# MiRaCLeXeoN/sduss

Measured on AMD Instinct MI355X. Metric: images/sec (node), SDXL 1024^2 50-step, fixed prompt, CFG, higher is better.
Workload: dtype bf16; 1 GPU; SDXL-base-1.0 UNet 1024x1024 50-step Euler, CFG 5.0, 4 requests/step (denoiser batch 8) per GPU, is_sliced=False, random-init weights of the real architecture (2.57 B params), one data-parallel replica per GPU, no collective; resolution=1024, steps_per_image=50

## Files before the change

include/mxdenoise.h:

```cpp
#ifndef MXDENOISE_H
#define MXDENOISE_H

#include <stddef.h>
#include <stdint.h>

#ifdef __cplusplus
extern "C" {
#endif

enum { MX_F32 = 0, MX_F16 = 1, MX_BF16 = 2 };

const char* mx_last_error(void);
int mx_version(void);
#define MX_PROF_KINDS 12
int mx_profile_enable(int on);
int mx_profile_collect(double* out);
int mx_profile_records(double* out, int max_records);

size_t mx_groupnorm_halo_workspace_bytes(int N, int C, int cpg);
int mx_groupnorm_halo(void* stream, const void* x, const void* gamma, const void* beta, void* y,
                      int N, int C, int H, int W, int cpg, double eps, int padding,
                      const int32_t* latent_offset, int n_latents, const int32_t* patch_map,
                      const int32_t* padding_idx, int dtype, void* workspace);
int mx_halo_only(void* stream, const void* x, void* y, int N, int C, int H, int W,
// ... 65 lines not shown
  float ln_eps;
  float* stats_out;
  const mx_gemm_seg* segs;
  int n_segs;
  int splitk;
  const float* ln_final;
  float* ln_final_out;
  unsigned* ln_final_cnt;
  float* gn_part_out;
  int cin_valid;
} mx_gemm_desc;

int mx_gemm(void* stream, const mx_gemm_desc* d);
int mx_gemm_launches(const mx_gemm_desc* d);
int mx_gemm_stats_slabs(const mx_gemm_desc* d);
int mx_gemm_ln_prefers_pass(const mx_gemm_desc* d);
int mx_gemm_ln_final_supported(const mx_gemm_desc* d);
int mx_gemm_gn_partials_supported(const mx_gemm_desc* d, int conv);
enum { MX_LN_ROUTES_PATCH_PARALLEL = 1, MX_LN_ROUTES_PATCH_CACHE = 2, MX_LN_ROUTES_TICKETS = 4 };
int mx_unet_ln_routes(int M, int C, int layers, int n_groups, int flags, int routes[4]);
enum { MX_FORM_TILE_GENERIC = 0, MX_FORM_TILE_256 = 1, MX_FORM_TILE_128 = 2, MX_FORM_PERSISTENT_256 = 3, MX_FORM_SMALL_M = 4, MX_FORM_CONV_SMALL_N = 5, MX_FORM_CONV_SMALL_CIN = 6 };
int mx_gemm_form(const mx_gemm_desc* d, int conv);
int mx_gemm_kernel_name(const mx_gemm_desc* d, int conv, int launch, char* buf, int cap);
int mx_gemm_kernel_names(char* buf, int cap);
int mx_attention_kernel_name(int B, int H, int Lq, int Lk, int ldo, int prescaled, int causal, int bias, int key_chunk, int force_cross, char* buf, int cap);
int mx_attention_kernel_names(char* buf, int cap);
#define MX_STATS_PITCH(slabs) (((slabs) + 3) & ~3)
int mx_row_stats(void* stream, const void* x, int ldx, float* stats, int M, int C);
int mx_conv3x3(void* stream, const mx_gemm_desc* d);
int mx_conv3x3_halo_serves(const mx_gemm_desc* d);
int mx_conv3x3_halo(void* stream, const mx_gemm_desc* d);
int mx_conv3x3_halfrow_serves(const mx_gemm_desc* d);
int mx_conv3x3_halfrow(void* stream, const mx_gemm_desc* d);
int mx_gemm_splitk(const mx_gemm_desc* d, int conv);
void mx_gemm_release_scratch(void* stream, int all);

#define MX_VT_POS(key) (((key) & ~12) | (((key) & 4) << 1) | (((key) & 8) >> 1))
#define MX_VT_LD(Lk) (((Lk) + 15) / 16 * 16)

int mx_attention(void* stream, const void* q, int ldq, const void* k, int ldk, const void* vt, int ldvt,
                 int64_t vt_batch_stride, void* o, int ldo, int B, int H, int Lq, int Lk, float scale);
#define MX_ATTN_QSCALE(scale) ((scale) * 1.4426950408889634f)
int mx_attention_prescaled(void* stream, const void* q, int ldq, const void* k, int ldk, const void* vt, int ldvt,
                           int64_t vt_batch_stride, void* o, int ldo, int B, int H, int Lq, int Lk);
int mx_attention_cross_prescaled(void* stream, const void* q, int ldq, const void* k, int ldk, const void* vt, int ldvt,
                                 int64_t vt_batch_stride, void* o, int ldo, int B, int H, int Lq, int Lk);
typedef struct mx_attn_problem {
  const void* q; const void* k; const void* vt; void* o;
  int64_t vt_batch_stride;
  int B, Lq, Lk, ldvt;
} mx_attn_problem;
int mx_attention_prescaled_grouped(void* stream, const mx_attn_problem* probs, int n, int ldq, int ldk, int ldo, int H);
int mx_attention_prescaled_bias(void* stream, const void* q, int ldq, const void* k, int ldk, const void* vt, int ldvt,
                                int64_t vt_batch_stride, void* o, int ldo, int B, int H, int Lq, int Lk, const float* bias, int ldb);
int mx_attention_prescaled_causal(void* stream, const void* q, int ldq, const void* k, int ldk, const void* vt, int ldvt,
                                  int64_t vt_batch_stride, void* o, int ldo, int B, int H, int L);

int mx_layernorm(void* stream, const void* x, void* y, const float* gamma, const float* beta,
                 int M, int C, float eps);

int mx_rmsnorm(void* stream, const void* x, void* y, const float* w, int M, int C, float eps);

int mx_layernorm_mod(void* stream, const void* x, void* y, void* y2, const float* scale, const float* shift,
                     const float* scale2, const float* shift2, int ldmod, int M, int C, int rows_per_batch, float eps);
int mx_layernorm_mod_grouped(void* stream, const void* x, void* y, void* y2, const float* scale, const float* shift, const float* scale2,
                             const float* shift2, int ldmod, int C, float eps, const int* batches, const int* rows_per_batch, int n);
// ... 378 lines not shown
```

sduss_amd/csrc/gemm_args.h:

```cpp
#pragma once
#include "common.h"
#include "../../include/mxdenoise.h"

namespace mx {

constexpr int kMaxSegs = MX_MAX_SEGS;
struct GemmSeg {
  const bf16_t* a; const bf16_t* a2; void* c; const bf16_t* residual; bf16_t* vt; const float* rowbias; const float* gate;
  const float* ln_stats; float* stats_out;
  int M, tile0, rows_per_batch, ldvt;
  int B, Hin, Win, Hout, Wout;
  int a_batch_rows, a_row_off, c_batch_rows, c_row_off;
};

struct GemmArgs {
  const bf16_t* a;
  const bf16_t* w;
  void* c;
  const float* bias;
  const float* rowbias;
  const bf16_t* residual;
  bf16_t* vt;
  int M, N, K;
  int lda, ldc, ldr, ldrb;
// ... 401 lines not shown
  const int band = local / band_tiles;
  const int r = local - band * band_tiles;
  const int rows = (mloc - band * MB) < MB ? (mloc - band * MB) : MB;
  tn = r / rows;
  tm = ((band * MB + (r - tn * rows)) << 3) + xcd;
}

__device__ __forceinline__ void lane_exchange_pair(float (&a)[4], float (&b)[4]) {
#pragma unroll
  for (int d = 0; d < 4; ++d) {
    unsigned x = __float_as_uint(a[d]), y = __float_as_uint(b[d]);
    auto r = __builtin_amdgcn_permlane32_swap(x, y, false, false);
    auto t = __builtin_amdgcn_permlane16_swap(r[0], r[1], false, false);
    a[d] = __uint_as_float(t[0]);
    b[d] = __uint_as_float(t[1]);
  }
}

__device__ __forceinline__ u32x4 lane_xor1(const u32x4 x) {
  u32x4 r;
#pragma unroll
  for (int d = 0; d < 4; ++d) r[d] = (unsigned)__builtin_amdgcn_update_dpp(0, (int)x[d], 0xB1, 0xF, 0xF, true);
  return r;
}

constexpr int EPI_F_QKV = 1;
constexpr int EPI_F_ACT = 2;
constexpr int EPI_F_ALL = 3;
constexpr int EPI_F_TANH = 4;
__host__ __device__ inline int gemm_epi_features(int flags) {
  const int acts = flags & (MX_EPI_SILU | MX_EPI_GELU | MX_EPI_GELU_TANH | MX_EPI_QUICK_GELU | MX_EPI_GEGLU_TANH);
  return ((flags & MX_EPI_QKV) ? EPI_F_QKV : 0) | (acts == 0 ? 0 : acts == MX_EPI_GELU_TANH ? EPI_F_TANH : EPI_F_ACT);
}
template <int NI, int MI, bool GEGLU, bool VEC = true, bool VPF = true, bool STATS = true, int FEAT = EPI_F_ALL, bool EMIT = STATS, bool RSTD_LOAD = false>
__device__ __forceinline__ void gemm_epilogue_regs(const GemmArgs& p, f32x4 (&acc)[NI][MI], const int m_wave0, const int wave_n0,
                                                   const int fr, const int fq, const float (&ln_rstd_a)[MI]) {
#pragma clang fp contract(off)
  constexpr int NIO = GEGLU ? NI / 2 : NI;
  constexpr int NP = NIO / 2;
  constexpr bool ODD = (NIO & 1) != 0;
  constexpr int DEPTH = MI <= 4 ? MI : 2;
  static_assert(!GEGLU || NI % 4 == 0, "GEGLU: hidden and gate halves must be whole pairs");
  const int flags = p.flags;
  constexpr bool ACT = (FEAT & EPI_F_ACT) != 0;
  constexpr bool TANH = (FEAT & (EPI_F_ACT | EPI_F_TANH)) != 0;
  const bool qkv = (FEAT & EPI_F_QKV) != 0 && (flags & MX_EPI_QKV) != 0;
  int seg_idx = 0, seg_grp = 0, seg_pos = 0;
  bool to_vt = false;
  if (qkv) {
    seg_idx = wave_n0 / p.seg;
    seg_grp = seg_idx / p.period;
    seg_pos = seg_idx - seg_grp * p.period;
    to_vt = seg_pos == p.period - 1;
  }
  const bool rms = qkv && (flags & MX_EPI_RMSNORM) && !to_vt;
  const float w_scale = (!rms && p.out_scale != 0.f && (!qkv || seg_pos == 0)) ? p.out_scale : 1.0f;
  const int col0 = GEGLU ? wave_n0 / 2 : qkv ? seg_grp * (p.period - 1) * p.seg + seg_pos * p.seg + (wave_n0 - seg_idx * p.seg) : wave_n0;
  const bool has_res = !GEGLU && p.residual != nullptr;
  const bool has_rb = VEC && !GEGLU && p.rowbias != nullptr, has_gate = VEC && !GEGLU && p.gate != nullptr;

  f32x4 bias_r[NI];
#pragma unroll
  for (int i = 0; i < NI; ++i) {
    bias_r[i] = f32x4{0.f, 0.f, 0.f, 0.f};
    if (p.bias && (GEGLU || i < NIO)) bias_r[i] = *reinterpret_cast<const f32x4*>(p.bias + wave_n0 + i * 16 + fq * 4);
  }
  f32x4 rmsw_r[NI];
  if (rms) {
    const float* w = seg_pos == 0 ? p.rms_wq : p.rms_wk;
// ... 27 lines not shown
#pragma unroll
          for (int i = 0; i < NIO; ++i) {
            const f32x4 t = STATS ? fma4(acc[i][j], rs, bias_r[i]) : acc[i][j] + bias_r[i];
#pragma unroll
            for (int q = 0; q < 4; ++q) dst[(long)(i * 16 + q) * p.ldvt] = f32_to_bf16(t[q]);
          }
        }
        rv += 16;
        if (rv >= rpb_v) { rv -= rpb_v; ++bv; }
      }
      return;
    }
  }
  const bool odd_lane = (fr & 1) != 0;
  const int rpb = p.rows_per_batch > 0 ? p.rows_per_batch : 0x7fffffff;
  const int cbr = p.c_batch_rows > 0 ? p.c_batch_rows : (p.rows_per_batch > 0 ? p.rows_per_batch : 0);
  const int cro = p.c_batch_rows > 0 ? p.c_row_off : 0;
  const int b_last = p.rows_per_batch > 0 ? (p.M - 1) / p.rows_per_batch : 0;
  const int r_last = p.M - 1 - b_last * (p.rows_per_batch > 0 ? p.rows_per_batch : 0);
  const int row_last = b_last * cbr + cro + r_last;
  const int mA0 = (m_wave0 + fr) & ~1;
  int row_a[MI], row_b[MI];
  int bo_walk = 0, ro_walk = 0;
  {
    int bA = p.rows_per_batch > 0 ? mA0 / p.rows_per_batch : 0;
    int rA = mA0 - bA * (p.rows_per_batch > 0 ? p.rows_per_batch : 0);
#pragma unroll
    for (int j = 0; j < MI; ++j) {
      int bB = bA, rB = rA + 1;
      if (rB >= rpb) { rB = 0; ++bB; }
      const int mA = mA0 + 16 * j;
      row_a[j] = mA < p.M ? bA * cbr + cro + rA : row_last;
      row_b[j] = mA + 1 < p.M ? bB * cbr + cro + rB : row_last;
      if constexpr (VEC) { if (j == 0) { bo_walk = odd_lane ? bB : bA; ro_walk = odd_lane ? rB : rA; } }
      rA += 16;
      if (rA >= rpb) { rA -= rpb; ++bA; }
    }
  }
  auto token = [&](int j) __attribute__((always_inline)) { return m_wave0 + j * 16 + fr; };
  auto row_own = [&](int j) __attribute__((always_inline)) { return odd_lane ? row_b[j] : row_a[j]; };
  const char* const res_base = reinterpret_cast<const char*>(p.residual);
  char* const c_base = reinterpret_cast<char*>(p.c);
  const unsigned ldr_b = (unsigned)p.ldr * 2u, ldc_b = (unsigned)p.ldc * 2u;
  auto res_at = [&](int row, int col) __attribute__((always_inline)) { return res_base + (unsigned long long)(unsigned)row * ldr_b + (unsigned)(col * 2); };
  auto c_at = [&](int row, int col) __attribute__((always_inline)) { return c_base + (unsigned long long)(unsigned)row * ldc_b + (unsigned)(col * 2); };
  auto store_c16 = [&](int row, int col, const u32x4 v) __attribute__((always_inline)) { *reinterpret_cast<u32x4*>(c_at(row, col)) = v; };
  auto store_c8 = [&](int row, int col, const u32x2 v) __attribute__((always_inline)) { *reinterpret_cast<u32x2*>(c_at(row, col)) = v; };

  auto load_res = [&](int j, int pr) __attribute__((always_inline)) -> u32x4 {
    if (!has_res) return u32x4{0u, 0u, 0u, 0u};
    return *reinterpret_cast<const u32x4*>(res_at(row_own(j), col0 + pr * 32 + fq * 8));
  };
  auto load_res_odd = [&](int j) __attribute__((always_inline)) -> u32x2 {
    if (!has_res) return u32x2{0u, 0u};
    return *reinterpret_cast<const u32x2*>(res_at(row_own(j), col0 + NP * 32 + fq * 4));
  };
  f32x4 rb_r[VEC ? NIO : 1], gate_r[VEC ? NIO : 1];
  auto load_batch_vectors = [&](int j) __attribute__((always_inline)) {
    if constexpr (VEC) {
      (void)j;
      const int bidx = bo_walk < b_last ? bo_walk : b_last;
      ro_walk += 16;
      if (ro_walk >= rpb) { ro_walk -= rpb; ++bo_walk; }
#pragma unroll
      for (int i = 0; i < NIO; ++i) {
        const int n = wave_n0 + i * 16 + fq * 4;
// ... 187 lines not shown
```

sduss_amd/csrc/gemm_dispatch.cpp:

```cpp
#include <algorithm>
#include <cstdlib>

#include <mutex>
#include <unordered_map>

#include "common.h"
#include "../../include/mxdenoise.h"
#include "gemm_args.h"
#include "gemm_forms.h"

namespace mx {

int launch_generic(hipStream_t s, const GemmArgs& a, int form);
int launch_v2(hipStream_t s, const GemmArgs& a, int form);
int launch_v5(hipStream_t s, const GemmArgs& a, int form);
int launch_v4(hipStream_t s, const GemmArgs& a, int form);
int launch_small_m(hipStream_t s, const GemmArgs& a, int form);
int launch_conv_small_n(hipStream_t s, const GemmArgs& a, int form);
int launch_conv_small_cin(hipStream_t s, const GemmArgs& a, int form);
bool small_m_serves(const mx_gemm_desc* d, bool conv);
int small_m_form(long N, long K, int flags);
bool conv_small_n_serves(const mx_gemm_desc* d);
bool conv_small_cin_serves(const mx_gemm_desc* d);

// ... 497 lines not shown
  for (const auto& s : kNotFaster) if (d->Win == s[0] && d->Cin == s[1] && d->N == s[2]) return 0;
  return conv_halo_lds_bytes(d->Win, false);
}

static int conv_halfrow_serves(const mx_gemm_desc* d) {
  if (!conv_staged_common(d) || d->Win != 128 || d->Hin % 4 != 0) return 0;
  return conv_halo_lds_bytes(d->Win, true);
}

static int run_conv_halo(void* stream, const mx_gemm_desc* d, bool half_rows) {
  MX_CHECK(d != nullptr, "conv3x3_halo: null descriptor");
  if (half_rows) MX_CHECK(conv_halfrow_serves(d) > 0, "conv3x3_halfrow: the descriptor is not served (mx_conv3x3_halfrow_serves); run mx_conv3x3");
  else MX_CHECK(conv_halo_serves(d) > 0, "conv3x3_halo: the descriptor is not served (mx_conv3x3_halo_serves); run mx_conv3x3");
  if (int rc = validate(d, true)) return rc;
  MX_CHECK(!d->stats_out && !d->ln_final_out, "conv3x3_halo: no row statistics");
  if (d->gn_part_out)
    MX_CHECK(!d->residual && (!d->rowbias || d->rows_per_batch % 64 == 0) && ((uintptr_t)d->gn_part_out & 15) == 0,
             "conv3x3_halo: gn_part_out needs an epilogue of bias (+ row bias) only and 16-byte alignment");
  GemmRoute r;
  r.bn = 160; r.rows = 256;
  GemmArgs a;
  fill_args(d, true, r, a);
  hipStream_t s = (hipStream_t)stream;
  if (prof_enabled()) {
    const double kk = 9.0 * d->Cin, Mt = (double)d->M;
    prof_begin(s, PROF_CONV_V2_160, 2.0 * Mt * (double)d->N * kk, 2.0 * (Mt * d->Cin + (double)d->N * d->K + Mt * d->N), d->M, d->N, (int)kk);
  }
  MX_CHECK(launch_conv_halo(s, a, d->rowbias != nullptr, half_rows) == 0, "conv3x3_halo: no instantiation for this image width");
  prof_end(s);
  MX_LAUNCH_CHECK();
  return 0;
}

}

extern "C" int mx_conv3x3_halo_serves(const mx_gemm_desc* d) { return mx::conv_halo_serves(d); }
extern "C" int mx_conv3x3_halo(void* stream, const mx_gemm_desc* d) { return mx::run_conv_halo(stream, d, false); }
extern "C" int mx_conv3x3_halfrow_serves(const mx_gemm_desc* d) { return mx::conv_halfrow_serves(d); }
extern "C" int mx_conv3x3_halfrow(void* stream, const mx_gemm_desc* d) { return mx::run_conv_halo(stream, d, true); }
extern "C" int mx_gemm(void* stream, const mx_gemm_desc* d) { return mx::run(stream, d, false); }
extern "C" int mx_conv3x3(void* stream, const mx_gemm_desc* d) { return mx::run(stream, d, true); }
extern "C" void mx_gemm_release_scratch(void* stream, int all) { mx::splitk_release((hipStream_t)stream, all != 0); }

extern "C" int mx_gemm_launches(const mx_gemm_desc* d) { mx::GemmPlan p; return mx::plan_of(d, false, p) ? p.n : 1; }
extern "C" int mx_gemm_form(const mx_gemm_desc* d, int conv) { mx::GemmPlan p; return mx::plan_of(d, conv != 0, p) ? (int)p.r[0].family : MX_FORM_TILE_GENERIC; }
extern "C" int mx_gemm_splitk(const mx_gemm_desc* d, int conv) { mx::GemmPlan p; return mx::plan_of(d, conv != 0, p) ? p.r[0].splitk : 0; }
extern "C" int mx_gemm_gn_partials_supported(const mx_gemm_desc* d, int conv) { mx::GemmPlan p; return mx::plan_of(d, conv != 0, p) && p.r[0].gn_part; }
extern "C" int mx_gemm_stats_slabs(const mx_gemm_desc* d) { mx::GemmPlan p; return mx::plan_of_variant(d, true, p) ? p.r[0].stats_slabs : 0; }
extern "C" int mx_gemm_ln_final_supported(const mx_gemm_desc* d) { mx::GemmPlan p; return mx::plan_of_variant(d, true, p) && p.r[0].ln_final_out; }
extern "C" int mx_gemm_ln_prefers_pass(const mx_gemm_desc* d) { mx::GemmPlan p; return mx::plan_of_variant(d, false, p) && p.r[0].bn == 256; }
extern "C" int mx_gemm_kernel_name(const mx_gemm_desc* d, int conv, int launch, char* buf, int cap) {
  mx::GemmPlan p;
  if (launch < 0 || !mx::plan_of(d, conv != 0, p)) return -1;
  if (launch >= p.n) return 0;
  if (p.r[launch].form < 0) return -1;
  return mx::copy_name(mx::kGemmKernelNames[p.r[launch].form], buf, cap);
}
extern "C" int mx_gemm_kernel_names(char* buf, int cap) { return mx::join_names(mx::kGemmKernelNames, mx::GK_COUNT, buf, cap); }
```

sduss_amd/csrc/unet_sdxl.cpp:

```cpp
#include <hip/hip_runtime.h>

#include <algorithm>
#include <cstring>
#include <functional>
#include <map>
#include <string>
#include <vector>

#include "../../include/mxdenoise.h"
#include "common.h"
#include "graph_cache.h"
#include "ln_route.h"
#include "patch_cache.h"
#include "plan_base.h"

namespace mx {
int launch_prep_latent(hipStream_t s, const void* in, int dtype, void* out, int B, int Cin, int HW, int CP);
int launch_nhwc_to_nchw(hipStream_t s, const void* in, void* out, int dtype, int B, int C, int HW, int ld);
int launch_time_embed(hipStream_t s, const float* timesteps, const void* text_embeds, const float* time_ids,
                      void* tsin, void* addin, int B, int d0, int text_dim, int da);
int launch_concat(hipStream_t s, const void* a, const void* b, void* out, long M, int C1, int C2);
size_t gn_workspace_exact(int B, int H, int W, int C, int patch);
int launch_sq_diff_partial(hipStream_t s, const void* a, const void* b, long elems_per_sample, int B, double* partial, const int* slot = nullptr);
int launch_gn_pp_partial(hipStream_t s, const void* x, int C1, const void* x2, int B, int H, int W, int C, int groups, void* workspace, double* sums);
// ... 2 lines not shown
                        const double* fresh_own = nullptr, int own_rank = 0);
}
extern "C" int mx_attention_prescaled_chunked(void* stream, const void* q, int ldq, const void* k, int ldk, const void* vt, int ldvt,
                                              int64_t vt_batch_stride, void* o, int ldo, int B, int H, int Lq, int Lk, int key_chunk,
                                              int64_t k_batch_stride, int64_t k_chunk_stride, int64_t vt_chunk_stride);

using mx::bf16_t;
using mx::LnVia;

struct mx_unet {
  mx_unet_config cfg;
  mx::WeightTable weights;
  mx::GraphCache graphs;
  mx::PinnedBuf skip_pin;
  std::map<std::vector<long>, std::vector<size_t>> pp_sizes;
  struct CtxEntry {
    uint64_t key = 0; int B = 0, ctx_len = 0; bool valid = false; uint64_t stamp = 0;
    std::vector<bf16_t*> k, vt; std::vector<size_t> k_bytes, vt_bytes;
    hipEvent_t ev = nullptr; hipStream_t last = nullptr; bool recorded = false;
  };
  uint64_t ctx_key = 0;
  std::vector<CtxEntry> ctx_store;
  uint64_t ctx_clock = 0;
  long ctx_hits = 0, ctx_misses = 0;
  void ctx_clear() {
    for (auto& e : ctx_store) {
      if (e.last) (void)hipStreamSynchronize(e.last);
      for (auto* q : e.k) if (q) (void)hipFree(q);
      for (auto* q : e.vt) if (q) (void)hipFree(q);
      if (e.ev) (void)hipEventDestroy(e.ev);
    }
    ctx_store.clear();
  }
  ~mx_unet() { ctx_clear(); }
};

namespace {

constexpr int kConvInPad = 64;

static std::vector<std::pair<int, int>> kv_widths(const mx_unet_config& c) {
  const int nlev = c.n_levels;
  std::vector<std::pair<int, int>> widths;
  auto add = [&](int dim, int n) { for (auto& wv : widths) if (wv.first == dim) { wv.second += n; return; } widths.push_back({dim, n}); };
  for (int i = 0; i < nlev; ++i) if (c.down_has_attn[i]) add(c.block_out_channels[i], c.layers_per_block * c.transformer_layers[i]);
  add(c.block_out_channels[nlev - 1], c.transformer_layers[nlev - 1]);
  for (int i = 0; i < nlev; ++i) { const int lv = nlev - 1 - i; if (c.down_has_attn[lv]) add(c.block_out_channels[lv], (c.layers_per_block + 1) * c.transformer_layers[lv]); }
  return widths;
}

struct RowStats { float* buf = nullptr; int slabs = 0; float* fin = nullptr; unsigned* cnt = nullptr; };
struct Linear {
  const bf16_t* a; int lda; std::string stem; void* c; int ldc; int M, N, K;
  const void* residual = nullptr; int ldr = 0; int flags = 0; float out_scale = 0.f;
  const bf16_t* a2 = nullptr; int lda2 = 0;
  const RowStats* ln = nullptr; LnVia ln_via = LnVia::Pass;
  RowStats* stats_out = nullptr; LnVia stats_via = LnVia::Pass;
  Linear& plus(const void* r, int ld) { residual = r; ldr = ld; return *this; }
  Linear& epilogue(int f) { flags = f; return *this; }
  Linear& scaled(float s) { out_scale = s; return *this; }
  Linear& concat(const bf16_t* x2, int ld2) { a2 = x2; lda2 = ld2; return *this; }
  Linear& folded_ln(const RowStats& st, LnVia via) { ln = &st; ln_via = via; return *this; }
  Linear& leaves_stats(RowStats& st, LnVia via) { stats_out = &st; stats_via = via; return *this; }
};
struct ConvIn { bf16_t* t = nullptr; bf16_t* padded = nullptr; };
struct Conv {
  ConvIn in; int Hin, Win, Cin; std::string prefix; bf16_t* out; int Cout;
  int stride = 1, up = 0, corner_patch = 0;
// ... 251 lines not shown
    d.corner_patch = c.corner_patch;
    d.M = gB[0] * d.Hout * d.Wout; d.N = Cout; d.K = 9 * Cin;
    d.rowbias = c.rowbias; d.ldrb = c.ldrb; d.rows_per_batch = d.Hout * d.Wout;
    d.residual = c.residual; d.ldr = Cout;
    mx_gemm_seg sg[MX_MAX_SEGS];
    if (ng > 1) {
      std::memset(sg, 0, sizeof(sg));
      long in0 = 0, out0 = 0;
      for (int g = 0; g < ng; ++g) {
        mx_gemm_seg& q = sg[g];
        q.B = gB[g]; q.Hin = ch[g]; q.Win = cw[g];
        q.Hout = ((ch[g] << up) + stride - 1) / stride; q.Wout = ((cw[g] << up) + stride - 1) / stride;
        q.M = gB[g] * q.Hout * q.Wout; q.rows_per_batch = q.Hout * q.Wout;
        q.a = x + in0 * Cin; q.c = c.out + out0 * Cout;
        q.residual = c.residual ? (const bf16_t*)c.residual + out0 * Cout : nullptr;
        q.rowbias = c.rowbias ? c.rowbias + (long)gb0[g] * c.ldrb : nullptr;
        in0 += (long)gB[g] * ch[g] * cw[g]; out0 += q.M;
      }
      d.segs = sg; d.n_segs = ng;
    }
    if (c.gn_part && c.gn_done && ng == 1 && mx_gemm_gn_partials_supported(&d, 1)) { d.gn_part_out = c.gn_part; *c.gn_done = true; }
    d.cin_valid = conv_cin_valid;
    if (mx_conv3x3_halo_serves(&d) && mx_gemm_form(&d, 1) == MX_FORM_TILE_256) {
      if (!ok()) return false;
      if (quiet()) return true;
      if (mx_conv3x3_halo(stream, &d)) return fail(std::string("conv3x3_halo: ") + mx_last_error());
      return true;
    }
    if (mx_conv3x3_halfrow_serves(&d) && mx_gemm_form(&d, 1) == MX_FORM_TILE_256) {
      if (!ok()) return false;
      if (quiet()) return true;
      if (mx_conv3x3_halfrow(stream, &d)) return fail(std::string("conv3x3_halfrow: ") + mx_last_error());
      return true;
    }
    return gemm(d, true);
  }
  bool groupnorm(const bf16_t* x, bf16_t* y, const std::string& prefix, int h, int wd, int C, float eps, bool silu, int patch,
                 const bf16_t* x2 = nullptr, int C1 = 0) {
    if (!ok()) return false;
    const size_t m = ar.mark();
    mx_gn_problem pr[MX_MAX_SEGS];
    long r0 = 0;
    for (int k = 0; k < ng; ++k) {
      pr[k].x = x + r0 * (x2 ? C1 : C); pr[k].x2 = x2 ? x2 + r0 * (C - C1) : nullptr; pr[k].y = y + r0 * C;
      pr[k].B = gB[k]; pr[k].H = ch[k]; pr[k].W = cw[k];
      r0 += (long)gB[k] * ch[k] * cw[k];
    }
    const size_t need = ng > 1 ? mx_groupnorm_nhwc_grouped_workspace_bytes(pr, ng, C) : mx::gn_workspace_exact(gB[0], h, wd, C, patch);
    void* ws = ar.alloc(need);
    if (!ws) return fail("workspace too small");
    const float* g = wf(prefix + ".weight", C); const float* b = wf(prefix + ".bias", C);
    if (ok() && !quiet()) {
      if (mx_groupnorm_nhwc_grouped(stream, pr, ng, x2 ? C1 : C, g, b, C, u->cfg.norm_num_groups, eps, silu ? 1 : 0, patch, ws))
        fail(std::string("groupnorm: ") + mx_last_error());
    }
    ar.release(m);
    return ok();
  }
  bool groupnorm_from_partials(const bf16_t* x, bf16_t* y, const std::string& prefix, int h, int wd, int C, float eps, bool silu, const float* part,
                               const float* add_bias, const float* add_rowbias, int ldrb) {
    if (!ok()) return false;
    const size_t m = ar.mark();
    void* ws = ar.alloc(mx::gn_workspace_exact(gB[0], h, wd, C, 0));
    if (!ws) return fail("workspace too small");
    const float* g = wf(prefix + ".weight", C); const float* b = wf(prefix + ".bias", C);
    if (ok() && !quiet()) {
// ... 729 lines not shown
extern "C" mx_unet* mx_unet_create(const mx_unet_config* cfg) {
  if (check_cfg(cfg)) return nullptr;
  mx_unet* u = new mx_unet();
  u->cfg = *cfg;
  return u;
}

extern "C" void mx_unet_destroy(mx_unet* u) { delete u; }

extern "C" int mx_unet_ln_routes(int M, int C, int layers, int n_groups, int flags, int routes[4]) {
  MX_CHECK(routes != nullptr && C > 0 && C % 64 == 0 && layers > 0 && n_groups >= 1 && n_groups <= MX_MAX_SEGS && M >= n_groups, "unet_ln_routes: bad arguments");
  const mx::LnRoutes r = mx::ln_routes(mx::LnRows::even(M, n_groups), C, layers, (flags & MX_LN_ROUTES_PATCH_PARALLEL) != 0, (flags & MX_LN_ROUTES_PATCH_CACHE) != 0,
                                       (flags & MX_LN_ROUTES_TICKETS) != 0);
  routes[0] = (int)r.norm1; routes[1] = (int)r.norm2; routes[2] = (int)r.norm3; routes[3] = r.norm3_from_merge ? 1 : 0;
  return 0;
}

extern "C" int mx_unet_set_context_key(mx_unet* u, uint64_t key) {
  MX_CHECK(u != nullptr, "unet_set_context_key: null handle");
  u->ctx_key = key;
  return 0;
}
extern "C" int mx_unet_context_stats(const mx_unet* u, long* hits, long* misses) {
  MX_CHECK(u != nullptr, "unet_context_stats: null handle");
  if (hits) *hits = u->ctx_hits;
  if (misses) *misses = u->ctx_misses;
  return 0;
}

extern "C" int mx_unet_set_weights(mx_unet* u, const void* blob, uint64_t blob_bytes, const mx_weight_entry* table, int n) {
  MX_CHECK(u != nullptr, "unet_set_weights: null handle");
  u->graphs.clear();
  u->ctx_clear();
  return u->weights.set("unet_set_weights", blob, blob_bytes, table, n);
}

extern "C" size_t mx_unet_workspace_bytes(const mx_unet* u, int batch, int H, int W, int ctx_len) {
  if (!u) return 0;
  size_t best = 0;
  const int div = 1 << (u->cfg.n_levels - 1);
  for (int gp : {0, 2 * div}) {
    if (gp > 0 && (H % gp != 0 || W % gp != 0 || gp >= H)) continue;
    size_t peak = 0;
    mx::ForwardCall c = dry_call(batch, H, W, ctx_len);
    c.gn_patch = gp; c.peak = &peak;
    if (forward_impl(u, c)) return 0;
    best = std::max(best, peak);
  }
  return best + 4096;
}

extern "C" int mx_unet_validate(const mx_unet* u, int batch, int H, int W, int ctx_len) {
  MX_CHECK(u && u->weights.blob, "unet_validate: weights not set");
  mx::ForwardCall c = dry_call(batch, H, W, ctx_len);
  c.lookup = true;
  return forward_impl(u, c);
}

extern "C" int mx_unet_forward(mx_unet* u, void* stream, const void* latents, int io_dtype, const float* timesteps,
                               const void* ehs, const void* text_embeds, const float* time_ids, void* out, int batch, int H,
                               int W, int ctx_len, int gn_patch, void* workspace, size_t workspace_bytes) {
  mx::ForwardCall c = forward_call(stream, io_dtype, timesteps, ehs, text_embeds, time_ids, ctx_len, workspace, workspace_bytes);
  c.latents = latents; c.out = out; c.batch = batch; c.H = H; c.W = W; c.gn_patch = gn_patch;
  return forward_impl(u, c);
}

extern "C" size_t mx_unet_workspace_bytes_mixed(const mx_unet* u, const mx_unet_group* groups, int n_groups, int ctx_len) {
// ... 233 lines not shown
```

sduss_amd/lib.py:

```python
from __future__ import annotations

import ctypes as C
import os
from typing import Optional

_HERE = os.path.dirname(os.path.abspath(__file__))
LIB_PATH = os.path.join(_HERE, "libmxdenoise.so")

MX_F32, MX_F16, MX_BF16 = 0, 1, 2
EPI_SILU, EPI_GEGLU, EPI_OUT_F32, EPI_QKV, EPI_GELU_TANH, EPI_RES_BCAST, EPI_RMSNORM, EPI_GELU, EPI_QUICK_GELU, EPI_GEGLU_TANH = 1, 2, 4, 8, 16, 32, 64, 128, 256, 512


class MxError(RuntimeError):
    """Raised for every non-zero status of the C ABI (the reference's launcher only printed
    cudaGetLastError and went on -- norm_silu_concat.cu:434-437; SURVEY.md section 8b asks to raise)."""


MAX_SEGS = 4


class GemmSeg(C.Structure):
    _fields_ = [
        ("a", C.c_void_p), ("a2", C.c_void_p), ("c", C.c_void_p), ("residual", C.c_void_p), ("vt", C.c_void_p), ("rowbias", C.c_void_p),
        ("gate", C.c_void_p), ("ln_stats", C.c_void_p), ("stats_out", C.c_void_p),
# ... 164 lines not shown
    _fields_ = [("kind", C.c_void_p), ("coef", C.c_void_p), ("hist", C.c_void_p)]


LORA_NO_VECTOR = (1 << 64) - 1
LORA_MAX_RANK = 512


class LoraTerm(C.Structure):
    _fields_ = [("w_off", C.c_uint64), ("N", C.c_int), ("K", C.c_int), ("row0", C.c_int), ("rows", C.c_int), ("up", C.c_void_p),
                ("down_t", C.c_void_p), ("R", C.c_int), ("scale", C.c_float), ("colsum_off", C.c_uint64), ("bias_off", C.c_uint64),
                ("dbias", C.c_void_p)]


class WeightEntry(C.Structure):
    _fields_ = [("name", C.c_char_p), ("offset", C.c_uint64), ("bytes", C.c_uint64)]


_vp, _i, _f, _d, _i64, _sz = C.c_void_p, C.c_int, C.c_float, C.c_double, C.c_int64, C.c_size_t
SYMBOLS = {
    "mx_last_error": (C.c_char_p, []),
    "mx_version": (_i, []),
    "mx_profile_enable": (_i, [_i]),
    "mx_profile_collect": (_i, [C.POINTER(C.c_double)]),
    "mx_profile_records": (_i, [C.POINTER(C.c_double), _i]),
    "mx_groupnorm_halo_workspace_bytes": (_sz, [_i, _i, _i]),
    "mx_groupnorm_halo": (_i, [_vp, _vp, _vp, _vp, _vp, _i, _i, _i, _i, _i, _d, _i, _vp, _i, _vp, _vp, _i, _vp]),
    "mx_halo_only": (_i, [_vp, _vp, _vp, _i, _i, _i, _i, _vp, _i]),
    "mx_gemm": (_i, [_vp, C.POINTER(GemmDesc)]),
    "mx_conv3x3": (_i, [_vp, C.POINTER(GemmDesc)]),
    "mx_conv3x3_halo": (_i, [_vp, C.POINTER(GemmDesc)]),
    "mx_conv3x3_halo_serves": (_i, [C.POINTER(GemmDesc)]),
    "mx_conv3x3_halfrow": (_i, [_vp, C.POINTER(GemmDesc)]),
    "mx_conv3x3_halfrow_serves": (_i, [C.POINTER(GemmDesc)]),
    "mx_gemm_stats_slabs": (_i, [C.POINTER(GemmDesc)]),
    "mx_gemm_ln_prefers_pass": (_i, [C.POINTER(GemmDesc)]),
    "mx_row_stats": (_i, [_vp, _vp, _i, _vp, _i, _i]),
    "mx_attention": (_i, [_vp, _vp, _i, _vp, _i, _vp, _i, _i64, _vp, _i, _i, _i, _i, _i, _f]),
    "mx_attention_prescaled": (_i, [_vp, _vp, _i, _vp, _i, _vp, _i, _i64, _vp, _i, _i, _i, _i, _i]),
    "mx_attention_cross_prescaled": (_i, [_vp, _vp, _i, _vp, _i, _vp, _i, _i64, _vp, _i, _i, _i, _i, _i]),
    "mx_layernorm": (_i, [_vp, _vp, _vp, _vp, _vp, _i, _i, _f]),
    "mx_groupnorm_nhwc_workspace_bytes": (_sz, [_i, _i, _i, _i]),
    "mx_groupnorm_nhwc": (_i, [_vp, _vp, _vp, _vp, _vp, _i, _i, _i, _i, _i, _f, _i, _i, _vp]),
    "mx_groupnorm_nhwc_cat": (_i, [_vp, _vp, _i, _vp, _vp, _vp, _vp, _i, _i, _i, _i, _i, _f, _i, _i, _vp]),
    "mx_attention_prescaled_grouped": (_i, [_vp, C.POINTER(AttnProblem), _i, _i, _i, _i, _i]),
    "mx_groupnorm_nhwc_grouped_workspace_bytes": (_sz, [C.POINTER(GnProblem), _i, _i]),
    "mx_groupnorm_nhwc_grouped": (_i, [_vp, C.POINTER(GnProblem), _i, _i, _vp, _vp, _i, _i, _f, _i, _i, _vp]),
    "mx_unet_workspace_bytes_mixed": (_sz, [_vp, C.POINTER(UNetGroup), _i, _i]),
    "mx_unet_forward_mixed": (_i, [_vp, _vp, C.POINTER(UNetGroup), _i, _i, _vp, _vp, _vp, _vp, _i, _i, _vp, _sz]),
    "mx_unet_forward_mixed_trace": (_i, [_vp, _vp, C.POINTER(UNetGroup), _i, _i, _vp, _vp, _vp, _vp, _i, _i, _vp, _sz, C.c_char_p, _vp, _sz]),
    "mx_mmdit_workspace_bytes_mixed": (_sz, [_vp, C.POINTER(UNetGroup), _i, _i]),
    "mx_mmdit_forward_mixed": (_i, [_vp, _vp, C.POINTER(UNetGroup), _i, _i, _vp, _vp, _vp, _i, _vp, _sz]),
    "mx_unet_create": (_vp, [C.POINTER(UNetConfigC)]),
    "mx_unet_destroy": (None, [_vp]),
    "mx_unet_set_context_key": (_i, [_vp, C.c_uint64]),
    "mx_unet_context_stats": (_i, [_vp, C.POINTER(C.c_long), C.POINTER(C.c_long)]),
    "mx_unet_set_weights": (_i, [_vp, _vp, C.c_uint64, C.POINTER(WeightEntry), _i]),
    "mx_unet_workspace_bytes": (_sz, [_vp, _i, _i, _i, _i]),
    "mx_unet_validate": (_i, [_vp, _i, _i, _i, _i]),
    "mx_unet_forward": (_i, [_vp, _vp, _vp, _i, _vp, _vp, _vp, _vp, _vp, _i, _i, _i, _i, _i, _vp, _sz]),
    "mx_forest_predict": (_i, [_vp, _vp, _vp, _vp, _vp, _vp, _i, _vp, _i, _i, _vp]),
    "mx_skip_counters_bytes": (_sz, [_i, _i, _i]),
    "mx_skip_decide_host": (_i, [C.POINTER(DeviceForestC), _i, _i, _i, _i, _vp, _vp, _vp, _vp, _vp, _vp, _vp, _vp, _vp]),
    "mx_skip_decide_device": (_i, [_vp, C.POINTER(SkipDecideArgs)]),
    "mx_pc_image_copy": (_i, [_vp, _vp, _vp, _vp, _i, _i, _i, _i64, _i, _vp, _i, _vp, _i64, _i]),
    "mx_pc_rows_load_stats": (_i, [_vp, _vp, _vp, _vp, _i, _i, _i, _i64, _vp, _vp, _vp, _f, _i64]),
    "mx_pc_gather": (_i, [_vp, _vp, _i, _i, _vp, _vp, _i, _vp, _i, _i, _i, _i, _i]),
# ... 184 lines not shown
```

Before: 1.493 images/s.

## Fuse nearest-2x upsample into 3x3 conv via per-phase folded weights

Adds a conv kernel for the upsampler convolutions that works on the low-resolution input. Nearest 2x upsampling followed by a 3x3 conv is rewritten as four output phases, each with pre-summed weights. The summed weights are packed once at weight load with bf16 hi/lo splits to keep precision, giving 7 slices instead of 9 and avoiding the upsampled intermediate. The new path costs extra device memory for packed weights, a special epilogue row mapping that scatters to interleaved output rows, and a separate kernel with its own pipelining.

```diff
diff --git a/include/mxdenoise.h b/include/mxdenoise.h
--- a/include/mxdenoise.h
+++ b/include/mxdenoise.h
@@ -121,6 +121,10 @@
 int mx_conv3x3_halo(void* stream, const mx_gemm_desc* d);
 int mx_conv3x3_halfrow_serves(const mx_gemm_desc* d);
 int mx_conv3x3_halfrow(void* stream, const mx_gemm_desc* d);
+size_t mx_conv3x3_up2_pack_bytes(int N, int Cin);
+int mx_conv3x3_up2_pack(void* stream, const void* w, int N, int Cin, void* wp);
+int mx_conv3x3_up2_serves(const mx_gemm_desc* d);
+int mx_conv3x3_up2(void* stream, const mx_gemm_desc* d, const void* wp);
 int mx_gemm_splitk(const mx_gemm_desc* d, int conv);
 void mx_gemm_release_scratch(void* stream, int all);
 
diff --git a/sduss_amd/csrc/conv_up2.hip b/sduss_amd/csrc/conv_up2.hip
--- /dev/null
+++ b/sduss_amd/csrc/conv_up2.hip
@@ -0,0 +1,258 @@
+#include "common.h"
+#include "../../include/mxdenoise.h"
+#include "gemm_args.h"
+#include "gemm_dma_loader.h"
+
+#include <type_traits>
+
+#ifndef MX_UP2_PHASE_SLOWEST
+#define MX_UP2_PHASE_SLOWEST 0
+#endif
+
+namespace mx {
+
+constexpr int UP2_BN = 160;
+constexpr int UP2_SLICES = 7;
+constexpr int UP2_WSTAGE_BYTES = UP2_BN * DMA_BK * 2;
+constexpr int UP2_ZERO_BYTES = 256;
+__host__ __device__ constexpr int up2_lines(int W) { return (256 / W + 2) * W; }
+__host__ __device__ constexpr int up2_xbuf_bytes(int W) { return up2_lines(W) * DMA_BK * 2; }
+__host__ __device__ constexpr int up2_lds_bytes(int W) { return 2 * up2_xbuf_bytes(W) + 3 * UP2_WSTAGE_BYTES + UP2_ZERO_BYTES; }
+__host__ __device__ constexpr int up2_slice_of_piece(int XN, int i) { return (i * 5) / (XN - 1); }
+__host__ __device__ constexpr int up2_pieces_in_slice(int XN, int T) {
+  int n = 0;
+  for (int i = 0; i < XN; ++i) n += up2_slice_of_piece(XN, i) == T ? 1 : 0;
+  return n;
+}
+
+__global__ __launch_bounds__(256) void up2_pack_kernel(const bf16_t* __restrict__ w, bf16_t* __restrict__ wp, const int N, const int Cin) {
+  const long idx = (long)blockIdx.x * 256 + threadIdx.x;
+  if (idx >= (long)N * Cin) return;
+  const int n = (int)(idx / Cin), c = (int)(idx - (long)n * Cin);
+  float t[3][3];
+#pragma unroll
+  for (int kh = 0; kh < 3; ++kh)
+#pragma unroll
+    for (int kw = 0; kw < 3; ++kw) t[kh][kw] = bf16_to_f32(w[(long)n * 9 * Cin + (long)(kh * 3 + kw) * Cin + c]);
+#pragma unroll
+  for (int ph = 0; ph < 4; ++ph) {
+    const int a = ph >> 1, b = ph & 1;
+    const int kho = a ? 2 : 0, kh0 = a ? 0 : 1, kh1 = kh0 + 1;
+    const int kwo = b ? 2 : 0, kw0 = b ? 0 : 1, kw1 = kw0 + 1;
+    const float sv = t[kho][kw0] + t[kho][kw1];
+    const float sh = t[kh0][kwo] + t[kh1][kwo];
+    const float sc = ((t[kh0][kw0] + t[kh0][kw1]) + t[kh1][kw0]) + t[kh1][kw1];
+    bf16_t* dst = wp + ((long)ph * N + n) * (UP2_SLICES * (long)Cin) + c;
+    const bf16_t vh = f32_to_bf16(sv), hh = f32_to_bf16(sh), ch = f32_to_bf16(sc);
+    dst[0] = f32_to_bf16(t[kho][kwo]);
+    dst[1 * (long)Cin] = vh; dst[2 * (long)Cin] = f32_to_bf16(sv - bf16_to_f32(vh));
+    dst[3 * (long)Cin] = hh; dst[4 * (long)Cin] = f32_to_bf16(sh - bf16_to_f32(hh));
+    dst[5 * (long)Cin] = ch; dst[6 * (long)Cin] = f32_to_bf16(sc - bf16_to_f32(ch));
+  }
+}
+
+int launch_up2_pack(hipStream_t s, const void* w, int N, int Cin, void* wp) {
+  const long n = (long)N * Cin;
+  hipLaunchKernelGGL(up2_pack_kernel, dim3((unsigned)((n + 255) / 256)), dim3(256), 0, s, (const bf16_t*)w, (bf16_t*)wp, N, Cin);
+  return 0;
+}
+
+template <int W>
+__global__ __launch_bounds__(512, 2) void conv_up2_kernel(const GemmArgs pk) {
+  constexpr int BN = UP2_BN, MI = 4, NI = BN / 32;
+  constexpr int LINES = up2_lines(W);
+  constexpr int XBUF = up2_xbuf_bytes(W);
+  constexpr int XN = LINES * 8 / 512;
+  constexpr int WCH = BN * 8, WI = 3;
+  constexpr int WRING = 2 * XBUF, ZERO = WRING + 3 * UP2_WSTAGE_BYTES;
+  static_assert(W == 32 || W == 64, "a tile is whole low-resolution rows of 32 or 64 pixels");
+  static_assert(up2_lds_bytes(W) <= 160 * 1024, "LDS of one workgroup");
+  static_assert(LINES * 8 % 512 == 0 && XBUF % 256 == 0, "whole DMA instructions; buffers keep the bank half of a line");
+  static_assert(up2_slice_of_piece(XN, XN - 1) == 5, "the last piece is issued one load phase before the chunk's last");
+  __shared__ __attribute__((aligned(256))) char smem[up2_lds_bytes(W)];
+
+  const GemmArgs& p = pk;
+  const int mt = p.M / 256, nt = p.N / BN;
+  int ph, bt;
+  {
+    const int b = blockIdx.x;
+    if (MX_UP2_PHASE_SLOWEST) { ph = b / (mt * nt); bt = b - ph * (mt * nt); }
+    else if ((mt & 7) != 0) { ph = b & 3; bt = b >> 2; }
+    else { const int local = b >> 3; ph = local & 3; bt = ((local >> 2) << 3) | (b & 7); }
+  }
+  int tm, tn;
+  gemm_tile_of_block(bt, mt, nt, p.xcd_map, tm, tn);
+  const int pa = ph >> 1, pb = ph & 1;
+  const int tid = threadIdx.x;
+  const int lane = tid & 63;
+  const int wave = __builtin_amdgcn_readfirstlane(tid >> 6);
+  const int wm = wave >> 1;
+  const int wn = wave & 1;
+  const bool group_b = wave >= 4;
+  const int cs = tid & 7;
+  const int nchunks = p.Cin / DMA_BK;
+  const char* zero = reinterpret_cast<const char*>(g_zero_page);
+
+  const int m0 = tm * 256, n0 = tn * BN;
+  const int hw = p.Hin * p.Win;
+  const int img = m0 / hw;
+  const int y0 = (m0 - img * hw) / W;
+  const char* xsrc[XN];
+#pragma unroll
+  for (int i = 0; i < XN; ++i) {
+    const int P = (i * 512 + tid) >> 3;
+    const int sr = P / W, x = P - sr * W;
+    const int iy = y0 - 1 + sr;
+    const bool ok = iy >= 0 && iy < p.Hin;
+    const long off = (((long)img * p.Hin + iy) * W + x) * (long)p.Cin * 2;
+    xsrc[i] = (ok ? reinterpret_cast<const char*>(p.a) + off : zero) + swz(P, cs) * 16;
+  }
+  const long w_row = UP2_SLICES * (long)p.Cin;
+  const char* wsrc[WI];
+#pragma unroll
+  for (int i = 0; i < WI; ++i) {
+    int q = i * 512 + tid;
+    if (q >= WCH) q -= WCH;
+    const int row = q >> 3;
+    wsrc[i] = reinterpret_cast<const char*>(p.w) + (((long)ph * p.N + n0 + row) * w_row + swz(row, cs) * 8) * 2;
+  }
+  const long w_slice_step = (long)p.Cin * 2, w_chunk_step = DMA_BK * 2 - (UP2_SLICES - 1) * (long)p.Cin * 2;
+
+  auto issue_x = [&](int buf, int i) __attribute__((always_inline)) {
+    glds16(xsrc[i], smem + buf * XBUF + (i * 512 + wave * 64) * 16);
+  };
+  auto advance_x = [&](int next_chunk) __attribute__((always_inline)) {
+#pragma unroll
+    for (int i = 0; i < XN; ++i) xsrc[i] = next_chunk < nchunks ? xsrc[i] + DMA_BK * 2 : zero + lane * 16;
+  };
+  auto issue_w = [&](int stage) __attribute__((always_inline)) {
+#pragma unroll
+    for (int i = 0; i < WI; ++i) {
+      const int qb = (i * 512 + wave * 64 >= WCH) ? i * 512 + wave * 64 - WCH : i * 512 + wave * 64;
+      glds16(wsrc[i], smem + WRING + stage * UP2_WSTAGE_BYTES + qb * 16);
+    }
+  };
+  auto step_w = [&](long step) __attribute__((always_inline)) {
+#pragma unroll
+    for (int i = 0; i < WI; ++i) wsrc[i] += step;
+  };
+  auto to_next_chunk_w = [&](bool last) __attribute__((always_inline)) {
+#pragma unroll
+    for (int i = 0; i < WI; ++i) wsrc[i] = last ? zero + lane * 16 : wsrc[i] + w_chunk_step;
+  };
+
+  const int fr = lane & 15;
+  const int fq = lane >> 4;
+  unsigned wrd[2];
+  unsigned xrd[3][2];
+  unsigned zrd[3][2];
+#pragma unroll
+  for (int ks = 0; ks < 2; ++ks) {
+    const int wrow = wn * (BN / 2) + fr;
+    wrd[ks] = (unsigned)(WRING + wrow * 128 + swz(wrow, ks * 4 + fq) * 16);
+#pragma unroll
+    for (int d = 0; d < 3; ++d) {
+      const int line = wm * 64 + fr + d - 1;
+      const int key = ((fr + d - 1) >> 1) & 7;
+      const int rel = line * 128 + ((ks * 4 + fq) ^ key) * 16;
+      xrd[d][ks] = (unsigned)rel;
+      zrd[d][ks] = (unsigned)(ZERO + (rel & 255));
+    }
+  }
+  const bool lane_left = fr == 0, lane_right = fr == 15;
+
+  if (tid < UP2_ZERO_BYTES / 16) *reinterpret_cast<u32x4*>(smem + ZERO + tid * 16) = u32x4{0u, 0u, 0u, 0u};
+
+#pragma unroll
+  for (int i = 0; i < XN; ++i) issue_x(0, i);
+  advance_x(1);
+  issue_w(0); step_w(w_slice_step);
+  issue_w(1); step_w(w_slice_step);
+  wait_vmcnt<WI>();
+
+  f32x4 acc[NI][MI];
+#pragma unroll
+  for (int i = 0; i < NI; ++i)
+#pragma unroll
+    for (int j = 0; j < MI; ++j) acc[i][j] = f32x4{0.f, 0.f, 0.f, 0.f};
+  float ln_rstd[MI];
+#pragma unroll
+  for (int j = 0; j < MI; ++j) ln_rstd[j] = 1.0f;
+  asm volatile("s_waitcnt lgkmcnt(0)" ::: "memory");
+  MX_BAR();
+  if (group_b) MX_BAR();
+
+  const unsigned yoff_o = (unsigned)((pa ? 2 : 0) * W * 128), yoff_s = (unsigned)(W * 128);
+  int stage = 0;
+
+  auto run = [&](auto pbc) __attribute__((always_inline)) {
+    constexpr bool PB = decltype(pbc)::value;
+    for (int cc = 0; cc < nchunks; ++cc) {
+      const int cur = cc & 1, nxt = cur ^ 1;
+      const unsigned xb = (unsigned)(cur * XBUF);
+      const bool last = cc + 1 == nchunks;
+      auto phase = [&](auto tc) __attribute__((always_inline)) {
+        constexpr int T = decltype(tc)::value;
+        constexpr int dx = (T == 0 || T == 3 || T == 4) ? (PB ? 1 : -1) : 0, d = dx + 1;
+        constexpr int NX = up2_pieces_in_slice(XN, T);
+        const unsigned xrow = xb + (T < 3 ? yoff_o : yoff_s);
+        const unsigned wst = (unsigned)(stage * UP2_WSTAGE_BYTES);
+        bf16x8 wf[2][NI], xf[2][MI];
+#pragma unroll
+        for (int ks = 0; ks < 2; ++ks) {
+#pragma unroll
+          for (int i = 0; i < NI; ++i) wf[ks][i] = *reinterpret_cast<const bf16x8*>(smem + wrd[ks] + wst + i * (16 * 128));
+#pragma unroll
+          for (int j = 0; j < MI; ++j) {
+            unsigned a = xrow + xrd[d][ks] + (unsigned)(j * (16 * 128));
+            if (dx == -1 && (j * 16) % W == 0) a = lane_left ? zrd[d][ks] : a;
+            if (dx == 1 && (j * 16 + 16) % W == 0) a = lane_right ? zrd[d][ks] : a;
+            xf[ks][j] = *reinterpret_cast<const bf16x8*>(smem + a);
+          }
+        }
+#pragma unroll
+        for (int i = 0; i < XN; ++i)
+          if (up2_slice_of_piece(XN, i) == T) issue_x(nxt, i);
+        const int st2 = stage == 0 ? 2 : stage - 1;
+        issue_w(st2);
+        stage = stage == 2 ? 0 : stage + 1;
+        if (T == 4) to_next_chunk_w(last);
+        else step_w(T > 4 && last ? 0 : w_slice_step);
+        if (T == UP2_SLICES - 1) advance_x(cc + 2);
+        wait_vmcnt<WI + NX>();
+        asm volatile("s_waitcnt lgkmcnt(0)" ::: "memory");
+        __builtin_amdgcn_sched_barrier(0);
+        MX_BAR();
+        __builtin_amdgcn_s_setprio(1);
+#pragma unroll
+        for (int ks = 0; ks < 2; ++ks)
+#pragma unroll
+          for (int i = 0; i < NI; ++i)
+#pragma unroll
+            for (int j = 0; j < MI; ++j) acc[i][j] = __builtin_amdgcn_mfma_f32_16x16x32_bf16(wf[ks][i], xf[ks][j], acc[i][j], 0, 0, 0);
+        __builtin_amdgcn_s_setprio(0);
+        MX_BAR();
+      };
+      phase(std::integral_constant<int, 0>{}); phase(std::integral_constant<int, 1>{}); phase(std::integral_constant<int, 2>{});
+      phase(std::integral_constant<int, 3>{}); phase(std::integral_constant<int, 4>{}); phase(std::integral_constant<int, 5>{});
+      phase(std::integral_constant<int, 6>{});
+    }
+  };
+  if (pb) run(std::true_type{}); else run(std::false_type{});
+  if (!group_b) MX_BAR();
+
+  gemm_epilogue_regs<NI, MI, false, false, true, true, 0, false, false, true>(p, acc, m0 + wm * 16 * MI, n0 + wn * (BN / 2), fr, fq, ln_rstd,
+                                                                              pa * 2 * W + pb);
+  wait_vmcnt<0>();
+}
+
+int conv_up2_lds_bytes(int width) { return width == 32 ? up2_lds_bytes(32) : width == 64 ? up2_lds_bytes(64) : 0; }
+
+int launch_conv_up2(hipStream_t s, const GemmArgs& a) {
+  const dim3 grid(4 * (a.M / 256) * (a.N / UP2_BN)), block(512);
+  if (a.Win == 32) { hipLaunchKernelGGL((conv_up2_kernel<32>), grid, block, 0, s, a); return 0; }
+  if (a.Win == 64) { hipLaunchKernelGGL((conv_up2_kernel<64>), grid, block, 0, s, a); return 0; }
+  return 1;
+}
+
+}
diff --git a/sduss_amd/csrc/gemm_args.h b/sduss_amd/csrc/gemm_args.h
--- a/sduss_amd/csrc/gemm_args.h
+++ b/sduss_amd/csrc/gemm_args.h
@@ -457,9 +457,10 @@
   const int acts = flags & (MX_EPI_SILU | MX_EPI_GELU | MX_EPI_GELU_TANH | MX_EPI_QUICK_GELU | MX_EPI_GEGLU_TANH);
   return ((flags & MX_EPI_QKV) ? EPI_F_QKV : 0) | (acts == 0 ? 0 : acts == MX_EPI_GELU_TANH ? EPI_F_TANH : EPI_F_ACT);
 }
-template <int NI, int MI, bool GEGLU, bool VEC = true, bool VPF = true, bool STATS = true, int FEAT = EPI_F_ALL, bool EMIT = STATS, bool RSTD_LOAD = false>
+template <int NI, int MI, bool GEGLU, bool VEC = true, bool VPF = true, bool STATS = true, int FEAT = EPI_F_ALL, bool EMIT = STATS, bool RSTD_LOAD = false,
+          bool UP2 = false>
 __device__ __forceinline__ void gemm_epilogue_regs(const GemmArgs& p, f32x4 (&acc)[NI][MI], const int m_wave0, const int wave_n0,
-                                                   const int fr, const int fq, const float (&ln_rstd_a)[MI]) {
+                                                   const int fr, const int fq, const float (&ln_rstd_a)[MI], const int up2_row0 = 0) {
 #pragma clang fp contract(off)
   constexpr int NIO = GEGLU ? NI / 2 : NI;
   constexpr int NP = NIO / 2;
@@ -553,6 +554,10 @@
       const int mA = mA0 + 16 * j;
       row_a[j] = mA < p.M ? bA * cbr + cro + rA : row_last;
       row_b[j] = mA + 1 < p.M ? bB * cbr + cro + rB : row_last;
+      if constexpr (UP2) {
+        row_a[j] = 4 * row_a[j] - 2 * (row_a[j] & (p.Win - 1)) + up2_row0;
+        row_b[j] = 4 * row_b[j] - 2 * (row_b[j] & (p.Win - 1)) + up2_row0;
+      }
       if constexpr (VEC) { if (j == 0) { bo_walk = odd_lane ? bB : bA; ro_walk = odd_lane ? rB : rA; } }
       rA += 16;
       if (rA >= rpb) { rA -= rpb; ++bA; }
diff --git a/sduss_amd/csrc/gemm_dispatch.cpp b/sduss_amd/csrc/gemm_dispatch.cpp
--- a/sduss_amd/csrc/gemm_dispatch.cpp
+++ b/sduss_amd/csrc/gemm_dispatch.cpp
@@ -553,8 +553,61 @@
   return 0;
 }
 
-}
-
+int launch_conv_up2(hipStream_t s, const GemmArgs& a);
+int launch_up2_pack(hipStream_t s, const void* w, int N, int Cin, void* wp);
+int conv_up2_lds_bytes(int width);
+
+static int conv_up2_serves(const mx_gemm_desc* d) {
+  if (!d || d->n_segs != 0 || d->stride != 1 || d->up != 1 || d->vhalo != 0 || d->corner_patch != 0) return 0;
+  if (d->Cin <= 0 || d->Cin % 64 != 0 || d->Cin > 8192 || d->K != 9 * d->Cin || d->cin_valid != 0) return 0;
+  if (d->N <= 0 || d->N % 160 != 0) return 0;
+  if (d->B <= 0 || d->Hin <= 0 || d->Win <= 0 || d->Hout != 2 * d->Hin || d->Wout != 2 * d->Win) return 0;
+  if ((long)d->B * d->Hout * d->Wout != d->M || (long)d->Hin * d->Win % 256 != 0) return 0;
+  if (d->flags != 0 || d->gate || d->out_scale != 0.f || d->splitk > 1) return 0;
+  if (d->rows_per_batch != 0 && d->rows_per_batch != d->Hout * d->Wout) return 0;
+  if (d->residual || d->rowbias || d->gn_part_out) return 0;
+  if (d->ldc % 8 != 0 || ((uintptr_t)d->c & 15) != 0) return 0;
+  return conv_up2_lds_bytes(d->Win);
+}
+
+static int run_conv_up2(void* stream, const mx_gemm_desc* d, const void* wp) {
+  MX_CHECK(d != nullptr, "conv3x3_up2: null descriptor");
+  MX_CHECK(conv_up2_serves(d) > 0, "conv3x3_up2: the descriptor is not served (mx_conv3x3_up2_serves); run mx_conv3x3");
+  if (int rc = validate(d, true)) return rc;
+  MX_CHECK(wp != nullptr && ((uintptr_t)wp & 15) == 0, "conv3x3_up2: the phase weights (mx_conv3x3_up2_pack) must be 16-byte aligned");
+  MX_CHECK(!d->stats_out && !d->ln_final_out, "conv3x3_up2: no row statistics");
+  MX_CHECK(4L * d->N * 7 * d->Cin < 2147483647L, "conv3x3_up2: phase weights exceed 32-bit indexing");
+  GemmRoute r;
+  r.bn = 160; r.rows = 256;
+  GemmArgs a;
+  fill_args(d, true, r, a);
+  a.M = d->B * d->Hin * d->Win; a.rows_per_batch = 0; a.w = (const bf16_t*)wp; a.K = 7 * d->Cin;
+  hipStream_t s = (hipStream_t)stream;
+  if (prof_enabled()) {
+    const double kk = 9.0 * d->Cin, Mt = (double)d->M;
+    prof_begin(s, PROF_CONV_V2_160, 2.0 * Mt * (double)d->N * kk, 2.0 * ((double)a.M * d->Cin + (double)d->N * d->K + Mt * d->N), d->M, d->N, (int)kk);
+  }
+  MX_CHECK(launch_conv_up2(s, a) == 0, "conv3x3_up2: no instantiation for this image width");
+  prof_end(s);
+  MX_LAUNCH_CHECK();
+  return 0;
+}
+
+static int run_up2_pack(void* stream, const void* w, int N, int Cin, void* wp) {
+  MX_CHECK(w && wp && N > 0 && Cin > 0, "conv3x3_up2_pack: bad arguments");
+  MX_CHECK((((uintptr_t)w | (uintptr_t)wp) & 15) == 0, "conv3x3_up2_pack: operand pointers must be 16-byte aligned");
+  MX_CHECK(4L * N * 7 * Cin < 2147483647L, "conv3x3_up2_pack: phase weights exceed 32-bit indexing");
+  MX_CHECK(launch_up2_pack((hipStream_t)stream, w, N, Cin, wp) == 0, "conv3x3_up2_pack: launch failed");
+  MX_LAUNCH_CHECK();
+  return 0;
+}
+
+}
+
+extern "C" size_t mx_conv3x3_up2_pack_bytes(int N, int Cin) { return N > 0 && Cin > 0 ? (size_t)4 * N * 7 * Cin * 2 : 0; }
+extern "C" int mx_conv3x3_up2_pack(void* stream, const void* w, int N, int Cin, void* wp) { return mx::run_up2_pack(stream, w, N, Cin, wp); }
+extern "C" int mx_conv3x3_up2_serves(const mx_gemm_desc* d) { return mx::conv_up2_serves(d); }
+extern "C" int mx_conv3x3_up2(void* stream, const mx_gemm_desc* d, const void* wp) { return mx::run_conv_up2(stream, d, wp); }
 extern "C" int mx_conv3x3_halo_serves(const mx_gemm_desc* d) { return mx::conv_halo_serves(d); }
 extern "C" int mx_conv3x3_halo(void* stream, const mx_gemm_desc* d) { return mx::run_conv_halo(stream, d, false); }
 extern "C" int mx_conv3x3_halfrow_serves(const mx_gemm_desc* d) { return mx::conv_halfrow_serves(d); }
diff --git a/sduss_amd/csrc/unet_sdxl.cpp b/sduss_amd/csrc/unet_sdxl.cpp
--- a/sduss_amd/csrc/unet_sdxl.cpp
+++ b/sduss_amd/csrc/unet_sdxl.cpp
@@ -58,8 +58,47 @@
     }
     ctx_store.clear();
   }
-  ~mx_unet() { ctx_clear(); }
+  struct Up2Pack { std::string prefix; int C = 0; void* wp = nullptr; };
+  std::vector<Up2Pack> up2;
+  void up2_clear() {
+    for (auto& e : up2) if (e.wp) (void)hipFree(e.wp);
+    up2.clear();
+  }
+  const void* up2_find(const std::string& prefix, int Cin, int Cout) const {
+    for (const auto& e : up2) if (e.C == Cin && e.C == Cout && e.prefix == prefix) return e.wp;
+    return nullptr;
+  }
+  int up2_build();
+  ~mx_unet() { ctx_clear(); up2_clear(); }
 };
+
+int mx_unet::up2_build() {
+  const bool had = !up2.empty();
+  if (had) (void)hipDeviceSynchronize();
+  up2_clear();
+  hipPointerAttribute_t at;
+  if (hipPointerGetAttributes(&at, weights.blob) != hipSuccess) { (void)hipGetLastError(); return 0; }
+  if (at.type != hipMemoryTypeDevice) return 0;
+  const int nlev = cfg.n_levels;
+  for (int i = 0; i + 1 < nlev; ++i) {
+    const int C = cfg.block_out_channels[nlev - 1 - i];
+    const std::string prefix = "up_blocks." + std::to_string(i) + ".upsamplers.0.conv";
+    mx_gemm_desc d; std::memset(&d, 0, sizeof(d));
+    d.c = (void*)(uintptr_t)16; d.ldc = C; d.B = 1; d.Hin = 8; d.Win = 32; d.Hout = 16; d.Wout = 64; d.Cin = C; d.N = C; d.K = 9 * C;
+    d.M = d.Hout * d.Wout; d.stride = 1; d.up = 1;
+    if (!mx_conv3x3_up2_serves(&d)) continue;
+    std::string e;
+    const void* w = weights.find(prefix + ".weight", (size_t)C * 9 * C * 2, e);
+    if (!w) continue;
+    Up2Pack pk; pk.prefix = prefix; pk.C = C;
+    MX_CHECK(hipMalloc(&pk.wp, mx_conv3x3_up2_pack_bytes(C, C)) == hipSuccess, "unet_set_weights: out of device memory for the upsamplers' phase weights");
+    up2.push_back(pk);
+    MX_HIP(hipDeviceSynchronize());
+    if (mx_conv3x3_up2_pack(nullptr, w, C, C, pk.wp)) return 1;
+    MX_HIP(hipStreamSynchronize(nullptr));
+  }
+  return 0;
+}
 
 namespace {
 
@@ -377,6 +416,14 @@
       if (quiet()) return true;
       if (mx_conv3x3_halfrow(stream, &d)) return fail(std::string("conv3x3_halfrow: ") + mx_last_error());
       return true;
+    }
+    if (up && mx_conv3x3_up2_serves(&d) && mx_gemm_form(&d, 1) == MX_FORM_TILE_256) {
+      if (const void* wp = u->up2_find(c.prefix, Cin, Cout)) {
+        if (!ok()) return false;
+        if (quiet()) return true;
+        if (mx_conv3x3_up2(stream, &d, wp)) return fail(std::string("conv3x3_up2: ") + mx_last_error());
+        return true;
+      }
     }
     return gemm(d, true);
   }
@@ -1172,7 +1219,8 @@
   MX_CHECK(u != nullptr, "unet_set_weights: null handle");
   u->graphs.clear();
   u->ctx_clear();
-  return u->weights.set("unet_set_weights", blob, blob_bytes, table, n);
+  if (int rc = u->weights.set("unet_set_weights", blob, blob_bytes, table, n)) return rc;
+  return u->up2_build();
 }
 
 extern "C" size_t mx_unet_workspace_bytes(const mx_unet* u, int batch, int H, int W, int ctx_len) {
diff --git a/sduss_amd/lib.py b/sduss_amd/lib.py
--- a/sduss_amd/lib.py
+++ b/sduss_amd/lib.py
@@ -220,6 +220,10 @@
     "mx_conv3x3_halo_serves": (_i, [C.POINTER(GemmDesc)]),
     "mx_conv3x3_halfrow": (_i, [_vp, C.POINTER(GemmDesc)]),
     "mx_conv3x3_halfrow_serves": (_i, [C.POINTER(GemmDesc)]),
+    "mx_conv3x3_up2_pack_bytes": (_sz, [_i, _i]),
+    "mx_conv3x3_up2_pack": (_i, [_vp, _vp, _i, _i, _vp]),
+    "mx_conv3x3_up2_serves": (_i, [C.POINTER(GemmDesc)]),
+    "mx_conv3x3_up2": (_i, [_vp, C.POINTER(GemmDesc), _vp]),
     "mx_gemm_stats_slabs": (_i, [C.POINTER(GemmDesc)]),
     "mx_gemm_ln_prefers_pass": (_i, [C.POINTER(GemmDesc)]),
     "mx_row_stats": (_i, [_vp, _vp, _i, _vp, _i, _i]),
```

Result: no change. 1.506 images/s (median of 6 runs) (+0.9%).
